# burchim/AVEC

Measured on AMD Instinct MI355X. Metric: AV utterances/sec fwd+bwd (audio T=400, video 100x88x88), higher is better.
Workload: dtype bf16

## Files before the change

avec_amd/csrc/api.hip:

```cpp
#include "common.h"
#include "avec_hip.h"
#include "vec.h"
#include "host_tables.h"
#include <stdarg.h>
#include <stdio.h>

static thread_local char g_err[512] = "";

void avec_set_error(const char* fmt, ...) {
  va_list ap; va_start(ap, fmt); vsnprintf(g_err, sizeof(g_err), fmt, ap); va_end(ap);
}
extern "C" const char* avec_last_error() { return g_err; }

static thread_local char g_kname[128] = "";
void avec_note_kernel(const char* fmt, ...) {
  va_list ap; va_start(ap, fmt); vsnprintf(g_kname, sizeof(g_kname), fmt, ap); va_end(ap);
}
extern "C" const char* avec_last_kernel() { return g_kname; }
extern "C" int avec_version() { return AVEC_ABI_VERSION; }
extern "C" int avec_struct_size(int which) {
  switch (which) {
    case 0: return (int)sizeof(avec_rows_t); case 1: return (int)sizeof(avec_epilogue_t); case 2: return (int)sizeof(avec_attn_t); case 3: return (int)sizeof(avec_tn_item_t);
    case 4: return (int)sizeof(avec_tn_batched_t); case 5: return (int)sizeof(avec_ln_item_t); case 6: return (int)sizeof(avec_fp8_item_t); case 7: return (int)sizeof(avec_wgrad3x3_item_t);
    case 8: return (int)sizeof(avec_ngram_t);
    default: return -1;
  }
}

static WsRegistry g_ws;
static LdsOptin g_lds;

extern "C" int avec_set_reduce_workspace(void* base, long long bytes) {
  int dev = 0; hipError_t e = hipGetDevice(&dev);
  AVEC_CHECK_ARG(e == hipSuccess && dev >= 0 && dev < WsRegistry::MAX_DEV, "set_reduce_workspace: no current device");
  AVEC_CHECK_ARG((base == nullptr && bytes == 0) || (base != nullptr && bytes >= (1 << 16) && ((size_t)base & 255) == 0),
                 "set_reduce_workspace: need a 256-byte aligned buffer of at least 64 KB (or NULL, 0 to unregister)");
  g_ws.set_default(dev, base, (size_t)bytes);
  return 0;
}
extern "C" int avec_set_reduce_workspace_stream(void* base, long long bytes, hipStream_t stream) {
  int dev = 0; hipError_t e = hipGetDevice(&dev);
  AVEC_CHECK_ARG(e == hipSuccess && dev >= 0 && dev < WsRegistry::MAX_DEV && base != nullptr && bytes >= (1 << 16) && ((size_t)base & 255) == 0, "set_reduce_workspace_stream: bad arguments");
  AVEC_CHECK_ARG(g_ws.set_stream(dev, stream, base, (size_t)bytes), "set_reduce_workspace_stream: at most %d stream-bound workspaces", WsRegistry::MAX_STREAMS);
  return 0;
}
ColWs avec_reduce_ws(size_t partial_floats, hipStream_t st) {
  int dev = 0; if (hipGetDevice(&dev) != hipSuccess) return ColWs{nullptr};
  return ColWs{(float*)g_ws.find(dev, st, partial_floats * sizeof(float))};
}

int avec_lds_optin_quiet(const void* kernel, size_t bytes) {
  if (bytes <= LdsOptin::FREE_BYTES) return 0;
  int dev = 0; if (hipGetDevice(&dev) != hipSuccess || dev < 0) return (int)hipErrorNoDevice;
  return g_lds.request(dev, kernel, bytes, [](const void* k, size_t n) {
    const hipError_t e = hipFuncSetAttribute(k, hipFuncAttributeMaxDynamicSharedMemorySize, (int)n);
    if (e != hipSuccess) (void)hipGetLastError();
    return (int)e;
// ... 9 lines not shown
```

avec_amd/lib.py:

```python
import ctypes
import os
import re

_HERE = os.path.dirname(os.path.abspath(__file__))
HEADER = os.path.join(os.path.dirname(_HERE), "include", "avec_hip.h")
LIB_PATH = os.environ.get("AVEC_LIB_PATH") or os.path.join(_HERE, "libavec_hip.so")

F32, BF16 = 0, 1
ROWS_PLAIN, ROWS_CONV_FWD, ROWS_CONV_BWD, ROWS_STEM3D = 0, 1, 2, 3
ACT_NONE, ACT_SWISH, ACT_RELU, ACT_GELU = 0, 1, 2, 3


class Rows(ctypes.Structure):
    _fields_ = [("ld", ctypes.c_longlong), ("rows_out", ctypes.c_int), ("rows_in", ctypes.c_int), ("step", ctypes.c_int),
                ("H", ctypes.c_int), ("W", ctypes.c_int), ("C", ctypes.c_int), ("KH", ctypes.c_int), ("KW", ctypes.c_int),
                ("stride", ctypes.c_int), ("pad", ctypes.c_int), ("OH", ctypes.c_int), ("OW", ctypes.c_int), ("T3", ctypes.c_int)]


class Epilogue(ctypes.Structure):
    _fields_ = [("out", ctypes.c_void_p), ("ldo", ctypes.c_longlong), ("out_f32", ctypes.c_int),
                ("out_pre", ctypes.c_void_p), ("ldpre", ctypes.c_longlong),
                ("bias", ctypes.c_void_p), ("act", ctypes.c_int),
                ("drop_p", ctypes.c_float), ("rng", ctypes.c_void_p), ("rng_stream", ctypes.c_uint),
                ("res", ctypes.c_void_p), ("ldres", ctypes.c_longlong), ("alpha", ctypes.c_float), ("res_act", ctypes.c_int),
# ... 14 lines not shown
                ("de", ctypes.c_void_p), ("ldde", ctypes.c_longlong), ("pbuf", ctypes.c_void_p), ("dsbuf", ctypes.c_void_p), ("ldt", ctypes.c_longlong), ("dsrel", ctypes.c_void_p), ("ldr", ctypes.c_longlong),
                ("B", ctypes.c_int), ("H", ctypes.c_int), ("T", ctypes.c_int), ("d", ctypes.c_int), ("scale", ctypes.c_float), ("Tk", ctypes.c_int)]


class TnItem(ctypes.Structure):
    _fields_ = [("P", ctypes.c_void_p), ("Q", ctypes.c_void_p), ("O", ctypes.c_void_p), ("p_colsum", ctypes.c_void_p),
                ("ldp", ctypes.c_longlong), ("ldq", ctypes.c_longlong), ("ldo", ctypes.c_longlong), ("M", ctypes.c_longlong),
                ("I", ctypes.c_int), ("J", ctypes.c_int), ("q_rows_out", ctypes.c_int), ("q_rows_in", ctypes.c_int), ("q_step", ctypes.c_int),
                ("reserved", ctypes.c_int)]


class TnBatched(ctypes.Structure):
    _fields_ = [("P", ctypes.c_void_p), ("ldp", ctypes.c_longlong), ("Q", ctypes.c_void_p), ("ldq", ctypes.c_longlong),
                ("O", ctypes.c_void_p), ("O_act", ctypes.c_void_p), ("ldo", ctypes.c_longlong),
                ("M", ctypes.c_longlong), ("I", ctypes.c_int), ("J", ctypes.c_int), ("nb_outer", ctypes.c_int), ("nb_inner", ctypes.c_int),
                ("strides6", ctypes.POINTER(ctypes.c_longlong))]


class LnItem(ctypes.Structure):
    _fields_ = [("dy", ctypes.c_void_p), ("x", ctypes.c_void_p), ("mean", ctypes.c_void_p), ("rstd", ctypes.c_void_p), ("dgamma", ctypes.c_void_p),
                ("dbeta", ctypes.c_void_p), ("M", ctypes.c_longlong), ("D", ctypes.c_int), ("dy_f32", ctypes.c_int)]


class Fp8Item(ctypes.Structure):
    _fields_ = [("src", ctypes.c_void_p), ("dst", ctypes.c_void_p), ("n", ctypes.c_longlong), ("slot", ctypes.c_int), ("K", ctypes.c_int), ("Kp", ctypes.c_int),
                ("reserved", ctypes.c_int)]


class WgradItem(ctypes.Structure):
    _fields_ = [("x", ctypes.c_void_p), ("dy", ctypes.c_void_p), ("dw", ctypes.c_void_p), ("images", ctypes.c_longlong), ("C", ctypes.c_int), ("H", ctypes.c_int),
                ("W", ctypes.c_int), ("reserved", ctypes.c_int)]


class NGram(ctypes.Structure):
    _fields_ = [("order", ctypes.c_int), ("V", ctypes.c_int), ("unigram", ctypes.c_void_p), ("ctx_cap", ctypes.c_longlong), ("ctx_key", ctypes.c_void_p),
                ("ctx_bo", ctypes.c_void_p), ("ctx_off", ctypes.c_void_p), ("ctx_cnt", ctypes.c_void_p), ("cont_tok", ctypes.c_void_p), ("cont_lp", ctypes.c_void_p)]


TN_GROUP_MAX, LN_GROUP_MAX, WGRAD_GROUP_MAX = 32, 40, 16
ABI_STRUCTS = (Rows, Epilogue, Attn, TnItem, TnBatched, LnItem, Fp8Item, WgradItem, NGram)


def _ctype(decl):
    decl = decl.strip()
    if "*" in decl or decl.startswith("hipStream_t"):
        return ctypes.c_void_p
    base = re.sub(r"\b[A-Za-z_][A-Za-z_0-9]*$", "", decl).strip() or decl
    base = base.replace("const", "").strip()
    return {"int": ctypes.c_int, "long long": ctypes.c_longlong, "float": ctypes.c_float, "unsigned": ctypes.c_uint,
            "void": None}[base]


def declared_functions(header=HEADER):
    txt = open(header).read()
    txt = re.sub(r"/\*.*?\*/", " ", txt, flags=re.S)
    out = {}
    for m in re.finditer(r"(?:^|\n)\s*(const char\*|long long|int)\s+(avec_[a-z0-9_]+)\s*\(([^;{]*?)\)\s*;", txt):
        ret, name, args = m.group(1), m.group(2), m.group(3)
        args = " ".join(args.split())
        argtypes = [] if args in ("", "void") else [_ctype(a) for a in args.split(",")]
        restype = {"int": ctypes.c_int, "long long": ctypes.c_longlong, "const char*": ctypes.c_char_p}[ret]
        out[name] = (restype, argtypes)
    return out


class _Lib:
    def __init__(self):
        self._dll = None

    def load(self):
        if self._dll is None:
            if not os.path.exists(LIB_PATH):
                raise RuntimeError("libavec_hip.so not found at %s -- build it with `python -m avec_amd.build` "
# ... 32 lines not shown
```

avec_amd/ops.py:

```python
import ctypes
import os

import torch

from . import fp8
from . import runtime as rt
from .lib import (ACT_GELU, ACT_NONE, ACT_RELU, ACT_SWISH, BF16, LN_GROUP_MAX, ROWS_CONV_BWD, ROWS_CONV_FWD, ROWS_PLAIN, ROWS_STEM3D, TN_GROUP_MAX, WGRAD_GROUP_MAX, Attn, Epilogue, LnItem, Rows, TnBatched, TnItem,
                  WgradItem, lib)

_byref = ctypes.byref


class KernelTimer:
    NAMES = {(0, ROWS_CONV_FWD): "gemm_nt<conv_fwd>", (0, ROWS_CONV_BWD): "gemm_nt<conv_bwd_data>", (0, ROWS_STEM3D): "gemm_nt<stem3d>",
             (0, ROWS_PLAIN): "gemm_nt<plain>", (1, ROWS_CONV_FWD): "gemm_tn<conv_wgrad>", (1, ROWS_STEM3D): "gemm_tn<stem3d_wgrad>",
             (1, ROWS_PLAIN): "gemm_tn<plain>", (2, 0): "conv3x3_slab<fwd>", (2, 1): "conv3x3_slab<bwd_data>", (2, 2): "conv3x3_slab<wgrad>"}

    def __init__(self):
        self.enabled = False
        self.records = []

    def reset(self, enabled):
        self.enabled, self.records = enabled, []

    def start(self):
        e = torch.cuda.Event(enable_timing=True)
        e.record()
        return e

    def stop(self, e0, key, flops, abytes=0.0):
        e1 = torch.cuda.Event(enable_timing=True)
        e1.record()
        name = lib.raw("avec_last_kernel")()
        self.records.append((key, flops, e0, e1, name.decode() if name else "", float(abytes)))

    def bracket_overhead_us(self, n=200):
        evs = []
        for _ in range(n):
            a, b = torch.cuda.Event(enable_timing=True), torch.cuda.Event(enable_timing=True)
            a.record(); b.record()
            evs.append((a, b))
# ... 147 lines not shown
    if res is not None:
        ep.res, ep.ldres, ep.res_act, ep.res_cls0 = res.data_ptr(), (N if ldres is None else ldres), int(res_act), int(res_cls0)
        if res_mask is not None:
            ep.res_mask = res_mask.data_ptr()
    ep.alpha = alpha
    if dact_z is not None:
        ep.dact_z, ep.ldz, ep.dact = dact_z.data_ptr(), N, dact
    ep.colsum, ep.stats = _p(colsum), _p(stats)
    if bnb is not None:
        ep.bnb_y, ep.ldby, ep.stats = bnb.y.data_ptr(), N, bnb.stats.data_ptr()
        if bnb.mask_z is not None:
            ep.dact_z, ep.ldz, ep.dact, ep.bnb_mask = bnb.mask_z.data_ptr(), N, 2, 0
        else:
            ep.bnb_ss, ep.bnb_mask = bnb.ss.data_ptr(), 1
    if rows is None:
        rows = rows_plain(K)
    ev = KERNEL_TIMER.start() if KERNEL_TIMER.enabled else None
    lib.gemm_nt(rt.dt() if dtype is None else dtype, A.data_ptr(), _byref(rows), mode, int(a_f32), W.data_ptr(),
                K if ldw is None else ldw, M, N, K, _byref(ep), rt.stream())
    if ev is not None:
        esz = A.element_size()
        KERNEL_TIMER.stop(ev, (0, mode), 2.0 * M * N * K if flops is None else flops,
                          ((M * K + N * K) * esz + M * N * (4 if out_f32 else esz)) if abytes is None else abytes)
    return out


DEFER_WGRAD = os.environ.get("AVEC_DEFER_WGRAD", "1") != "0"
_TN_WHY = False
_TN_FLUSH_AT = TN_GROUP_MAX
_DEFER = {"queues": {}, "task": -1}


class _PendingGrads:
    __slots__ = ("stream", "tn", "ln", "keep", "flops", "cw", "cw_flops", "cw64", "cw64_flops")

    def __init__(self, stream):
        self.stream, self.tn, self.ln, self.keep, self.flops = stream, [], [], [], 0.0
        self.cw, self.cw_flops = [], 0.0
        self.cw64, self.cw64_flops = [], 0.0


def _in_backward():
    return DEFER_WGRAD and torch._C._current_graph_task_id() != -1


def reset_backward_state():
    for q in _DEFER["queues"].values():
        q.tn, q.ln, q.keep, q.flops, q.cw, q.cw_flops, q.cw64, q.cw64_flops = [], [], [], 0.0, [], 0.0, [], 0.0
    _DEFER["task"] = -1
    _PREP_READY["task"], _PREP_READY["m"] = -1, {}
    _LN2_READY["task"], _LN2_READY["m"] = -1, {}
    for ent in _POS_CACHE.values():
        ent[1].de_all, ent[1].remaining = None, ent[1].L


def _pending():
    st = torch.cuda.current_stream()
    q = _DEFER["queues"].get(st.cuda_stream)
    if q is None:
        q = _DEFER["queues"][st.cuda_stream] = _PendingGrads(st)
    task = torch._C._current_graph_task_id()
    if _DEFER["task"] != task:
        if _DEFER["task"] != -1:
            for old in _DEFER["queues"].values():
                old.tn, old.ln, old.keep, old.flops, old.cw, old.cw_flops, old.cw64, old.cw64_flops = [], [], [], 0.0, [], 0.0, [], 0.0
        _DEFER["task"] = task
        torch.autograd.Variable._execution_engine.queue_callback(_flush_at_end)
    return q


def _launch_pending(q, part=None):
    cur = torch.cuda.current_stream()
    if cur.cuda_stream != q.stream.cuda_stream:
        for t in q.keep:
            t.record_stream(cur)
    if q.tn and part in (None, "tn"):
        ev = KERNEL_TIMER.start() if KERNEL_TIMER.enabled else None
        for i in range(0, len(q.tn), TN_GROUP_MAX):
            chunk = q.tn[i:i + TN_GROUP_MAX]
            lib.gemm_tn_grouped(BF16, (TnItem * len(chunk))(*chunk), len(chunk), rt.stream())
        if ev is not None:
            KERNEL_TIMER.stop(ev, (1, ROWS_PLAIN), q.flops, sum(2.0 * it.M * (it.I + it.J) + 4.0 * it.I * it.J for it in q.tn))
        q.tn, q.flops = [], 0.0
    if q.ln and part in (None, "ln"):
        for i in range(0, len(q.ln), LN_GROUP_MAX):
            chunk = q.ln[i:i + LN_GROUP_MAX]
            lib.layernorm_param_grads_grouped(rt.dt(), (LnItem * len(chunk))(*chunk), len(chunk), rt.stream())
        q.ln = []
    if q.cw and part in (None, "cw"):
        ev = KERNEL_TIMER.start() if KERNEL_TIMER.enabled else None
        for i in range(0, len(q.cw), WGRAD_GROUP_MAX):
            chunk = q.cw[i:i + WGRAD_GROUP_MAX]
            lib.wgrad3x3_c128_grouped((WgradItem * len(chunk))(*chunk), len(chunk), rt.stream())
        if ev is not None:
            KERNEL_TIMER.stop(ev, (2, 2), q.cw_flops, sum(2.0 * 2 * it.images * it.H * it.W * it.C + 4.0 * 9 * it.C * it.C for it in q.cw))
        q.cw, q.cw_flops = [], 0.0
    if q.cw64 and part in (None, "cw"):
        ev = KERNEL_TIMER.start() if KERNEL_TIMER.enabled else None
        for i in range(0, len(q.cw64), WGRAD_GROUP_MAX):
            chunk = q.cw64[i:i + WGRAD_GROUP_MAX]
            lib.wgrad3x3_c64_grouped((WgradItem * len(chunk))(*chunk), len(chunk), rt.stream())
        if ev is not None:
            KERNEL_TIMER.stop(ev, (2, 2), q.cw64_flops, sum(2.0 * 2 * it.images * it.H * it.W * it.C + 4.0 * 9 * it.C * it.C for it in q.cw64))
        q.cw64, q.cw64_flops = [], 0.0
    if not q.tn and not q.ln and not q.cw and not q.cw64:
        q.keep = []


def flush_param_grads(all_streams=False):
    if all_streams:
        for q in list(_DEFER["queues"].values()):
            _launch_pending(q)
        return
    q = _DEFER["queues"].get(torch.cuda.current_stream().cuda_stream)
    if q is not None:
        _launch_pending(q)


def _flush_at_end():
    _DEFER["task"] = -1
    flush_param_grads(all_streams=True)


def gemm_tn(P, Q, O, M, I, J, *, ldp=None, q_rows=None, q_mode=ROWS_PLAIN, q_f32=False, ldo=None, dtype=None, p_colsum=None, side=False):
    if q_rows is None:
        q_rows = rows_plain(J)
    if side and q_mode == ROWS_PLAIN and q_f32 and CAST_DEFER and dtype is None and rt.compute_dtype() == "bf16" and _in_backward() and Q.dim() == 2 and Q.dtype == torch.float32:
        Qb = empty((Q.shape[0], J), rt.act_dtype(), Q)
        lib.cast_rows(rt.dt(), Q.data_ptr(), q_rows.ld, Qb.data_ptr(), J, Q.shape[0], J, rt.stream())
        Q, q_f32, q_rows = Qb, False, rows_plain(J, q_rows.rows_out, q_rows.rows_in, q_rows.step)
    if side and q_mode == ROWS_PLAIN and not q_f32 and dtype is None and rt.compute_dtype() == "bf16" and _in_backward():
        it = TnItem()
        it.P, it.Q, it.O, it.p_colsum = P.data_ptr(), Q.data_ptr(), O.data_ptr(), _p(p_colsum)
        it.ldp, it.ldq, it.ldo, it.M, it.I, it.J = (I if ldp is None else ldp), q_rows.ld, (J if ldo is None else ldo), M, I, J
        it.q_rows_out, it.q_rows_in, it.q_step = q_rows.rows_out, q_rows.rows_in, q_rows.step
        if lib.raw("avec_gemm_tn_grouped_ok")(BF16, _byref(it)) and _chunk_readable(P, it.ldp, I, M) and _chunk_readable(Q, it.ldq, J, M):
            q = _pending()
            q.tn.append(it)
# ... 997 lines not shown
        ctx.saved = (grad, M)
        return mean

    @staticmethod
    def backward(ctx, dloss):
        grad, M = ctx.saved
        out = torch.empty_like(grad)
        lib.scale_by_scalar(grad.data_ptr(), dloss.float().contiguous().data_ptr(), 1.0 / M, out.data_ptr(), grad.numel(), rt.stream())
        return out, None, None


def conv2d_fwd(x, weight, N, H, W, Cin, stride, stats=None):
    Cout, KH, KW = weight.shape[0], weight.shape[2], weight.shape[3]
    pad = (KH - 1) // 2
    OH, OW = (H - 1) // stride + 1, (W - 1) // stride + 1
    M = N * OH * OW
    sh = rt.shadow(weight)
    y = empty((M, Cout), rt.act_dtype(), x)
    if _slab_conv(H, W, Cin, Cout, KH, KW, stride):
        ev = KERNEL_TIMER.start() if KERNEL_TIMER.enabled else None
        lib.conv3x3_c64(x.data_ptr(), sh.fwd.data_ptr(), y.data_ptr(), None, _p(stats), N, H, W, 0, rt.stream())
        if ev is not None:
            KERNEL_TIMER.stop(ev, (2, 0), 2.0 * M * Cout * KH * KW * Cin, 2.0 * (N * H * W * Cin + Cout * KH * KW * Cin + M * Cout))
        return y, OH, OW
    gemm_nt(x, sh.fwd, y, M, Cout, KH * KW * Cin, rows=rows_conv(H, W, Cin, KH, KW, stride, pad, OH, OW), mode=ROWS_CONV_FWD, stats=stats,
            abytes=2.0 * (N * H * W * Cin + Cout * KH * KW * Cin + M * Cout))
    return y, OH, OW


SLAB_CONV = True
SLAB_WGRAD128 = True
SHORTCUT_SUBGRID = True
GROUP_WGRAD128 = True


def _slab_conv(H, W, Cin, Cout, KH, KW, stride):
    return SLAB_CONV and rt.act_dtype() == torch.bfloat16 and bool(lib.raw("avec_conv3x3_c64_supported")(H, W, Cin, Cout, KH, KW, stride))


class BnbFuse:
    __slots__ = ("y", "ss", "mask_z", "stats", "done")

    def __init__(self, y, ss, mask_z, C):
        self.y, self.ss, self.mask_z, self.done = y, ss, mask_z, False
        self.stats = rt.zeros_scratch(BNState.NREP * 2 * C, y.device)


BNB_FUSE = False


def conv2d_bwd(dy, x, weight, N, H, W, Cin, stride, OH, OW, need_dx=True, dx_res=None, bnb=None, dx_res_cls0=False, dx_res_mask=None):
    Cout, KH, KW = weight.shape[0], weight.shape[2], weight.shape[3]
    pad = (KH - 1) // 2
    M = N * OH * OW
    sh = rt.shadow(weight)
    if _slab_conv(H, W, Cin, Cout, KH, KW, stride) and H * (W + 1) <= 512:
        if GROUP_WGRAD128 and _in_backward():
            it = WgradItem()
            it.x, it.dy, it.dw, it.images, it.C, it.H, it.W = x.data_ptr(), dy.data_ptr(), grad_of(weight).data_ptr(), N, Cin, H, W
            q = _pending()
            q.cw64.append(it)
            q.keep += [x, dy]
            q.cw64_flops += 2.0 * M * Cout * KH * KW * Cin
        else:
            ev = KERNEL_TIMER.start() if KERNEL_TIMER.enabled else None
            lib.wgrad3x3_c64(x.data_ptr(), dy.data_ptr(), grad_of(weight).data_ptr(), N, H, W, rt.stream())
            if ev is not None:
                KERNEL_TIMER.stop(ev, (2, 2), 2.0 * M * Cout * KH * KW * Cin)
    elif SLAB_CONV and SLAB_WGRAD128 and rt.act_dtype() == torch.bfloat16 and bool(lib.raw("avec_wgrad3x3_c128_supported")(H, W, Cin, Cout, KH, KW, stride)):
        if GROUP_WGRAD128 and _in_backward():
            it = WgradItem()
            it.x, it.dy, it.dw, it.images, it.C, it.H, it.W = x.data_ptr(), dy.data_ptr(), grad_of(weight).data_ptr(), N, Cin, H, W
            q = _pending()
            q.cw.append(it)
            q.keep += [x, dy]
            q.cw_flops += 2.0 * M * Cout * KH * KW * Cin
        else:
            ev = KERNEL_TIMER.start() if KERNEL_TIMER.enabled else None
            lib.wgrad3x3_c128(x.data_ptr(), dy.data_ptr(), grad_of(weight).data_ptr(), N, Cin, H, W, rt.stream())
            if ev is not None:
                KERNEL_TIMER.stop(ev, (2, 2), 2.0 * M * Cout * KH * KW * Cin)
    else:
        gemm_tn(dy, x, grad_of(weight), M, Cout, KH * KW * Cin, q_rows=rows_conv(H, W, Cin, KH, KW, stride, pad, OH, OW), q_mode=ROWS_CONV_FWD, side=True)
    if not need_dx:
        return None
    dx = empty((N * H * W, Cin), rt.act_dtype(), dy)
    if _slab_conv(H, W, Cin, Cout, KH, KW, stride):
        ev = KERNEL_TIMER.start() if KERNEL_TIMER.enabled else None
        if dx_res_mask is not None:
            lib.conv3x3_c64_res_masked(dy.data_ptr(), sh.bwd.data_ptr(), dx.data_ptr(), dx_res.data_ptr(), dx_res_mask.data_ptr(), N, H, W, 1, rt.stream())
        else:
            lib.conv3x3_c64(dy.data_ptr(), sh.bwd.data_ptr(), dx.data_ptr(), _p(dx_res), None, N, H, W, 1, rt.stream())
        if ev is not None:
            KERNEL_TIMER.stop(ev, (2, 1), 2.0 * N * H * W * Cin * KH * KW * Cout, 2.0 * (2 * N * H * W * Cin + Cout * KH * KW * Cin + M * Cout))
        return dx
    fuse = bnb if (bnb is not None and BNB_FUSE and rt.act_dtype() == torch.bfloat16 and Cin % 4 == 0) else None
    gemm_nt(dy, sh.bwd, dx, N * H * W, Cin, KH * KW * Cout, rows=rows_conv(H, W, Cout, KH, KW, stride, pad, OH, OW), mode=ROWS_CONV_BWD,
            res=dx_res, res_act=True, flops=2.0 * N * OH * OW * Cout * KH * KW * Cin, bnb=fuse, res_cls0=dx_res_cls0, res_mask=dx_res_mask,
            abytes=2.0 * (N * H * W * Cin * (2 if dx_res is not None else 1) + Cout * KH * KW * Cin + M * Cout))
    if fuse is not None:
        fuse.done = True
    return dx


RES_MASK = True


def res_mask_ok(H, W, Cin, Cout, stride):
    if rt.act_dtype() != torch.bfloat16 or stride != 1 or Cin != Cout:
        return False
    return _slab_conv(H, W, Cin, Cout, 3, 3, 1) or (Cin >= 128 and Cin % 32 == 0 and W <= 31)


class ResNetBlockFn(torch.autograd.Function):
# ... 467 lines not shown
```

include/avec_hip.h:

```cpp
#ifndef AVEC_HIP_H
#define AVEC_HIP_H
#include <stdint.h>
#ifdef __HIPCC__
#include <hip/hip_runtime.h>
#else
typedef struct ihipStream_t* hipStream_t;
#endif
#ifdef __cplusplus
extern "C" {
#endif

#define AVEC_F32 0
#define AVEC_BF16 1
#define AVEC_ABI_VERSION 4
#define AVEC_STAT_REPLICAS 64

int avec_version(void);
int avec_struct_size(int which);
const char* avec_last_error(void);
const char* avec_last_kernel(void);
int avec_set_reduce_workspace(void* base, long long bytes);
int avec_set_reduce_workspace_stream(void* base, long long bytes, hipStream_t stream);

enum { AVEC_ROWS_PLAIN = 0, AVEC_ROWS_CONV_FWD = 1, AVEC_ROWS_CONV_BWD = 2 };
// ... 166 lines not shown
                        const float* count_ptr, float count, int phase, float* dw, float* dbias, float* dgamma, float* dbeta,
                        int B, int n_mels, int F, int C, hipStream_t stream);
int avec_stem_im2col(int dtype, const float* video, void* A, long long clips, int T, int H, int W, int ldk, hipStream_t stream);
int avec_stem3d_supported(long long clips, int T, int H, int W);
int avec_stem3d_fwd(const float* video, const void* w_shadow, int ldw, const float* bias, void* y, float* stats, long long clips, int T, int H, int W, hipStream_t stream);
int avec_stem3d_wgrad(const float* video, const void* dy, float* dw, long long clips, int T, int H, int W, hipStream_t stream);
int avec_stem3p_supported(long long clips, int T, int H, int W);
int avec_stem3p_fwd(const void* video_bf16, const void* w_shadow, const float* bias, const float* gamma, void* zp, unsigned char* idx, float* stats,
                    long long clips, int T, int H, int W, hipStream_t stream);
int avec_stem3p_reduce(void* dpool, const void* zp, const float* ss, float* dstats, long long frames, int PH, int PW, hipStream_t stream);
int avec_stem3p_wgrad_supported(long long clips, int T, int H, int W);
int avec_stem3p_wgrad(const void* video_bf16, const void* w_shadow, const float* bias, const void* dpool_masked, const unsigned char* idx, const float* ss,
                      const float* gamma, const float* dstats, const float* count_ptr, float count, float* dw, float* dgamma, float* dbeta,
                      long long clips, int T, int H, int W, hipStream_t stream);
int avec_stem3p_dz(const void* video_bf16, const void* w_shadow, const float* bias, const void* dpool_masked, const unsigned char* idx, const float* ss,
                   const float* gamma, const float* dstats, const float* count_ptr, float count, void* dz, float* dgamma, float* dbeta,
                   long long clips, int T, int H, int W, hipStream_t stream);
int avec_stem_pool_fwd(int dtype, const void* y, const float* ss, void* out, unsigned char* idx, void* ymax, long long frames, int H, int W, int C, hipStream_t stream);
int avec_stem_pool_bwd_reduce_pooled(int dtype, const void* dpool, const unsigned char* idx, const void* ymax, const float* ss, float* dstats,
                                     long long frames, int H, int W, int C, hipStream_t stream);
int avec_stem_pool_bwd(int dtype, const void* dpool, const unsigned char* idx, const void* y, const float* ss, const float* gamma, float* dstats,
                       const float* count_ptr, float count, int phase, void* dy, float* dgamma, float* dbeta, long long frames, int H, int W, int C, hipStream_t stream);

int avec_conv3x3_c64_supported(int H, int W, int Cin, int Cout, int KH, int KW, int stride);
int avec_conv3x3_c64(const void* x, const void* w, void* y, const void* res, float* stats, long long images, int H, int W, int flip, hipStream_t stream);
int avec_conv3x3_c64_res_masked(const void* x, const void* w, void* y, const void* res, const unsigned char* res_mask, long long images, int H, int W, int flip, hipStream_t stream);
int avec_wgrad3x3_c64(const void* x, const void* dy, float* dw, long long images, int H, int W, hipStream_t stream);
int avec_wgrad3x3_c128_supported(int H, int W, int Cin, int Cout, int KH, int KW, int stride);
int avec_wgrad3x3_c128(const void* x, const void* dy, float* dw, long long images, int C, int H, int W, hipStream_t stream);
#define AVEC_WGRAD_GROUP_MAX 16
typedef struct { const void* x; const void* dy; float* dw; long long images; int C, H, W, reserved; } avec_wgrad3x3_item_t;
int avec_wgrad3x3_c128_grouped(const avec_wgrad3x3_item_t* items, int n, hipStream_t stream);
int avec_wgrad3x3_c64_grouped(const avec_wgrad3x3_item_t* items, int n, hipStream_t stream);

int avec_video_input(const unsigned char* clips, const long long* clip_off, const int* geom, const int* masks, int max_masks, int channels, const float* lut, float mean, float stdv,
                     int mean_frame, float* out, float* frame_ws, int B, int Tout, int OH, int OW, hipStream_t stream);

long long avec_ctc_workspace_floats(int B, int T, int Lmax);
int avec_ctc_loss(const float* logits, const long long* in_lens, const long long* targets, const long long* tgt_lens, float* nll, float* mean_out,
                  float* grad, float* workspace, int B, int T, int V, int Lmax, int blank, int zero_infinity, hipStream_t stream);
int avec_ctc_loss_multi_fits(int T, int V, int Lmax);
int avec_ctc_loss_multi(int n_heads, const float* const* logits, const long long* const* in_lens, const int* T, float* const* nll, float* const* mean_out, float* const* grad,
                        const long long* targets, const long long* tgt_lens, const float* weights, float* total, int B, int V, int Lmax, int blank, int zero_infinity, hipStream_t stream);
int avec_scale_by_scalar(const float* g, const float* scalar_dev, float mul, float* out, long long n, hipStream_t stream);
int avec_scale_by_scalar_multi(int n_tensors, const float* const* g, float* const* out, const long long* numel, const float* mul, const float* scalar_dev, hipStream_t stream);
int avec_softmax_ce(const float* logits, const long long* targets, long long ignore_index, float* loss, float* mean_out, float* grad, long long M, int V, hipStream_t stream);
int avec_len_affine(const long long* in, long long* out, int n, long long sub, long long div, long long add, hipStream_t stream);
int avec_argmax_rows(const float* x, long long* out, long long M, int V, hipStream_t stream);

typedef struct avec_ngram {
  int order;
  int V;
  const float* unigram;
  long long ctx_cap;
  const unsigned long long* ctx_key;
  const float* ctx_bo;
  const int* ctx_off;
  const int* ctx_cnt;
  const int* cont_tok;
  const float* cont_lp;
} avec_ngram_t;
long long avec_ctc_beam_workspace_bytes(int B, int T, int W);
int avec_ctc_beam_search(const float* logits, const long long* lengths, int B, int T, int V, int W, float inv_tmp, const avec_ngram_t* lm, float alpha, float beta,
                         float oov_logprob, void* workspace, long long workspace_bytes, int* tokens, int* out_len, float* score, float* ctc_logp, hipStream_t stream);
int avec_ngram_rows(const avec_ngram_t* lm, const int* ctx, const int* ctx_len, int n, int max_len, float oov_logprob, float* rows, hipStream_t stream);
long long avec_ctc_align_workspace_bytes(int B, int T, int Lmax);
// ... 26 lines not shown
```

Before: 1869.

## Add grouped MFMA weight-gradient kernel for stride-2 3x3 convolutions

Adds a dedicated bf16 MFMA kernel that computes weight gradients for stride-2 3x3 convs (ResNet downsample layers at 22/11/6 spatial sizes). It loads dy and the four parity-class x windows into double-buffered LDS with global_load_lds, applies boundary masks per tap, and atomically accumulates into fp32 dw. The grads are deferred and batched into a single grouped launch that balances tiles across 256 blocks. This replaces the generic implicit-GEMM TN path for these layers, at the cost of atomics and a narrow supported geometry.

```diff
diff --git a/avec_amd/csrc/api.hip b/avec_amd/csrc/api.hip
--- a/avec_amd/csrc/api.hip
+++ b/avec_amd/csrc/api.hip
@@ -22,7 +22,7 @@
   switch (which) {
     case 0: return (int)sizeof(avec_rows_t); case 1: return (int)sizeof(avec_epilogue_t); case 2: return (int)sizeof(avec_attn_t); case 3: return (int)sizeof(avec_tn_item_t);
     case 4: return (int)sizeof(avec_tn_batched_t); case 5: return (int)sizeof(avec_ln_item_t); case 6: return (int)sizeof(avec_fp8_item_t); case 7: return (int)sizeof(avec_wgrad3x3_item_t);
-    case 8: return (int)sizeof(avec_ngram_t);
+    case 8: return (int)sizeof(avec_ngram_t); case 9: return (int)sizeof(avec_wgrad_s2_item_t);
     default: return -1;
   }
 }
diff --git a/avec_amd/csrc/wgrad_s2.hip b/avec_amd/csrc/wgrad_s2.hip
--- /dev/null
+++ b/avec_amd/csrc/wgrad_s2.hip
@@ -0,0 +1,251 @@
+#include "common.h"
+#include "avec_hip.h"
+#include "wgrad_s2_plan.h"
+
+#include <stdlib.h>
+
+namespace {
+
+typedef __attribute__((ext_vector_type(16))) float ws_f32x16;
+typedef __attribute__((ext_vector_type(8))) __bf16 ws_bf16x8;
+typedef short ws_v4s __attribute__((ext_vector_type(4)));
+typedef __attribute__((address_space(3))) char ws_lds;
+
+constexpr int WS_DYB = WS2_BM * WS2_BCO * 2;
+constexpr int WS_XWB = WS2_WR * WS2_BCI * 2;
+constexpr int WS_TBL = WS_DYB + 4 * WS_XWB;
+constexpr int WS_STAGE = (WS_TBL + 5 * WS2_BM * 2 + 1023) / 1024 * 1024;
+constexpr size_t WS_LDS = 2 * (size_t)WS_STAGE;
+static_assert(WS_LDS <= 160 * 1024, "two stages must fit the LDS");
+constexpr int WS_XI = WS_XWB / 1024, WS_DYI = WS_DYB / 1024;
+constexpr int WS_WAVES = 8, WS_WCO = 4;
+constexpr int WS_NF = WS2_BCO / 32 / WS_WCO;
+static_assert(WS_NF >= 1 && WS2_BCI / 32 * WS_WCO == WS_WAVES, "wave grid");
+
+struct Ws2Item { const char* x; const char* dy; float* dw; Ws2Geom g; int tiles, kinds, nci, L; };
+struct Ws2Group { Ws2Item it[AVEC_WGRAD_GROUP_MAX]; long long cum[AVEC_WGRAD_GROUP_MAX + 1]; int n; };
+
+__device__ __forceinline__ void ws_glds16(unsigned voff, const void* sbase, unsigned lds_dst_uniform) {
+  unsigned keep;
+  asm volatile("s_mov_b32 %0, m0\n\ts_mov_b32 m0, %3\n\ts_nop 0\n\tglobal_load_lds_dwordx4 %1, %2\n\ts_mov_b32 m0, %0" : "=&s"(keep) : "v"(voff), "s"(sbase), "s"(lds_dst_uniform) : "memory");
+}
+__device__ __forceinline__ uint2 ws_tr(const ws_lds* p) {
+  typedef __attribute__((address_space(3))) ws_v4s* lp_t;
+  return __builtin_bit_cast(uint2, __builtin_amdgcn_ds_read_tr16_b64_v4i16((lp_t)p));
+}
+typedef unsigned ws_u32x4 __attribute__((ext_vector_type(4)));
+__device__ __forceinline__ ws_u32x4 ws_ld128(const ws_lds* p) { return *(const __attribute__((address_space(3))) ws_u32x4*)p; }
+struct WsFrag { uint2 lo, hi; };
+__device__ __forceinline__ void ws_and(WsFrag& f, const ws_u32x4& m) { f.lo.x &= m.x; f.lo.y &= m.y; f.hi.x &= m.z; f.hi.y &= m.w; }
+__device__ __forceinline__ ws_f32x16 ws_mma(const WsFrag& a, const WsFrag& b, ws_f32x16 c) {
+  chunk16 fa, fb; fa.w[0] = a.lo.x; fa.w[1] = a.lo.y; fa.w[2] = a.hi.x; fa.w[3] = a.hi.y; fb.w[0] = b.lo.x; fb.w[1] = b.lo.y; fb.w[2] = b.hi.x; fb.w[3] = b.hi.y;
+  return __builtin_amdgcn_mfma_f32_32x32x16_bf16(__builtin_bit_cast(ws_bf16x8, fa), __builtin_bit_cast(ws_bf16x8, fb), c, 0, 0, 0);
+}
+
+struct WsMasks { ws_u32x4 v, t, l, b, r; };
+template <bool ODD>
+__device__ __forceinline__ void ws_load_masks(WsMasks& m, const ws_lds* const tb, const int s) {
+  m.v = ws_ld128(tb + 32 * s); m.t = ws_ld128(tb + 128 + 32 * s); m.l = ws_ld128(tb + 256 + 32 * s);
+  if (ODD) { m.b = ws_ld128(tb + 384 + 32 * s); m.r = ws_ld128(tb + 512 + 32 * s); }
+}
+
+template <bool ODD>
+__device__ __forceinline__ void ws2_run(const char* const xb, const char* const dyb, float* const dw, const Ws2Geom& g, const int nci, ws_lds* const lds, const unsigned lds0,
+                                        const int kind, const int tb, const int te) {
+  const int tid = threadIdx.x, lane = tid & 63, wave = __builtin_amdgcn_readfirstlane(tid >> 6);
+  const int cog = kind / nci, cig = kind - cog * nci, co0 = cog * WS2_BCO, ci0 = cig * WS2_BCI;
+  const int wco = wave % WS_WCO, wci = wave / WS_WCO;
+  const int g4 = lane >> 4, t = lane & 15;
+
+  unsigned aA[WS_NF], aB[9];
+  {
+    const int krow = 8 * (g4 >> 1) + (t >> 2);
+#pragma unroll
+    for (int f = 0; f < WS_NF; ++f) aA[f] = (unsigned)(krow * 256 + (((2 * (WS_NF * wco + f) + (g4 & 1)) ^ (2 * (krow & 3))) << 5) + (t & 3) * 8);
+#pragma unroll
+    for (int tap = 0; tap < 9; ++tap) {
+      const int kh = tap / 3, kw = tap % 3, cls = ((kh + 1) & 1) * 2 + ((kw + 1) & 1);
+      const int row = WS2_HALO + krow - (kh == 0 ? g.OW : 0) - (kw == 0 ? 1 : 0);
+      aB[tap] = (unsigned)(WS_DYB + cls * WS_XWB + row * 128 + (((2 * wci + (g4 & 1)) ^ (2 * ((row >> 1) & 1))) << 5) + (t & 3) * 8);
+    }
+  }
+  const unsigned tblo = (unsigned)(WS_TBL + 16 * (lane >> 5));
+
+  ws_f32x16 acc[WS_NF][9];
+#pragma unroll
+  for (int f = 0; f < WS_NF; ++f)
+#pragma unroll
+    for (int j = 0; j < 9; ++j)
+#pragma unroll
+      for (int r = 0; r < 16; ++r) acc[f][j][r] = 0.f;
+
+  auto issue_stage = [&](const int tile, const int par) {
+    const unsigned m0 = (unsigned)tile * WS2_BM, st = (unsigned)par * WS_STAGE;
+#pragma unroll
+    for (int k = 0; k < WS_DYI / WS_WAVES; ++k) {
+      const int q = wave + WS_WAVES * k, row = 4 * q + (lane >> 4), lu = (lane & 15) ^ (4 * (lane >> 4));
+      unsigned p = m0 + (unsigned)row; p = p < g.P ? p : g.P - 1;
+      ws_glds16((p * (unsigned)g.Cout + (unsigned)(co0 + lu * 8)) * 2u, dyb, lds0 + st + (unsigned)q * 1024u);
+    }
+#pragma unroll
+    for (int k = 0; k < (WS_XI + WS_WAVES - 1) / WS_WAVES; ++k) {
+      const int idx = wave + WS_WAVES * k;
+      if (idx < WS_XI) {
+        int row, lu; ws2_x_slot(idx, lane, row, lu);
+        const unsigned base = ws2_x_base(g, m0, row, lu, ci0);
+#pragma unroll
+        for (int cls = 0; cls < 4; ++cls) ws_glds16(ws2_x_issue(g, base, cls), xb, lds0 + st + (unsigned)(WS_DYB + cls * WS_XWB) + (unsigned)idx * 1024u);
+      }
+    }
+    if (tid < WS2_BM) {
+      const unsigned p = m0 + (unsigned)tid, pc = p < g.P ? p : g.P - 1;
+      const unsigned tt = ws2_div(pc, g.OW), j = pc - tt * (unsigned)g.OW, i = tt - ws2_div(tt, g.OH) * (unsigned)g.OH;
+      typedef __attribute__((address_space(3))) unsigned short lds_u16;
+      lds_u16* const tb_ = (lds_u16*)(lds + st + WS_TBL);
+      tb_[tid] = p < g.P ? 0xffffu : 0u;
+      tb_[WS2_BM + tid] = i > 0 ? 0xffffu : 0u;
+      tb_[2 * WS2_BM + tid] = j > 0 ? 0xffffu : 0u;
+      tb_[3 * WS2_BM + tid] = (int)(2 * i + 1) < g.H ? 0xffffu : 0u;
+      tb_[4 * WS2_BM + tid] = (int)(2 * j + 1) < g.W ? 0xffffu : 0u;
+    }
+  };
+
+  int par = 0;
+  issue_stage(tb, 0);
+  for (int tile = tb; tile < te; ++tile, par ^= 1) {
+    asm volatile("s_waitcnt vmcnt(0) lgkmcnt(0)" ::: "memory");
+    __builtin_amdgcn_s_barrier();
+    asm volatile("" ::: "memory");
+    if (tile + 1 < te) issue_stage(tile + 1, par ^ 1);
+    const ws_lds* const sb = lds + par * WS_STAGE;
+    constexpr int NK = WS2_BM / 16, NSEQ = NK * 9, AHEAD = 3;
+    const ws_lds* const tbl = sb + tblo;
+    WsFrag A[2][WS_NF], B[4]; ws_u32x4 mv[2], mt, ml, mb, mr;
+    auto load_a = [&](const int s) {
+#pragma unroll
+      for (int f = 0; f < WS_NF; ++f) { A[s & 1][f].lo = ws_tr(sb + aA[f] + s * 4096); A[s & 1][f].hi = ws_tr(sb + aA[f] + s * 4096 + 1024); }
+      mv[s & 1] = ws_ld128(tbl + 32 * s);
+    };
+    auto load_b = [&](const int n) { const int s = n / 9, tap = n % 9; B[n & 3].lo = ws_tr(sb + aB[tap] + s * 2048); B[n & 3].hi = ws_tr(sb + aB[tap] + s * 2048 + 512); };
+    load_a(0);
+    mt = ws_ld128(tbl + 128); ml = ws_ld128(tbl + 256);
+#pragma unroll
+    for (int n = 0; n < AHEAD; ++n) load_b(n);
+#pragma unroll
+    for (int n = 0; n < NSEQ; ++n) {
+      const int s = n / 9, tap = n % 9, kh = tap / 3, kw = tap % 3;
+      if (n + AHEAD < NSEQ) load_b(n + AHEAD);
+      if (tap == 4 && s + 1 < NK) load_a(s + 1);
+      if (ODD && tap == 0) { mb = ws_ld128(tbl + 384 + 32 * s); mr = ws_ld128(tbl + 512 + 32 * s); }
+      if (tap == 0) {
+#pragma unroll
+        for (int f = 0; f < WS_NF; ++f) ws_and(A[s & 1][f], mv[s & 1]);
+      }
+      WsFrag& b = B[n & 3];
+      if (kh == 0) ws_and(b, mt);
+      if (kw == 0) ws_and(b, ml);
+      if (ODD && kh == 2) ws_and(b, mb);
+      if (ODD && kw == 2) ws_and(b, mr);
+#pragma unroll
+      for (int f = 0; f < WS_NF; ++f) acc[f][tap] = ws_mma(A[s & 1][f], b, acc[f][tap]);
+      if (tap == 2 && s + 1 < NK) mt = ws_ld128(tbl + 128 + 32 * (s + 1));
+      if (tap == 6 && s + 1 < NK) ml = ws_ld128(tbl + 256 + 32 * (s + 1));
+      __builtin_amdgcn_sched_barrier(0);
+    }
+  }
+#pragma unroll
+  for (int f = 0; f < WS_NF; ++f)
+#pragma unroll
+    for (int j = 0; j < 9; ++j)
+#pragma unroll
+      for (int r = 0; r < 16; ++r) {
+        const int co = co0 + (wco * WS_NF + f) * 32 + (r & 3) + 8 * (r >> 2) + 4 * (lane >> 5), ci = ci0 + wci * 32 + (lane & 31);
+        atomicAdd(dw + ((long long)co * 9 + j) * g.Cin + ci, acc[f][j][r]);
+      }
+  __builtin_amdgcn_s_barrier();
+}
+
+__global__ __launch_bounds__(WS_WAVES * 64) void wgrad3x3_s2_grouped_kernel(Ws2Group grp) {
+  extern __shared__ __attribute__((aligned(16))) char smem[];
+  ws_lds* const lds = (ws_lds*)smem;
+  const unsigned lds0 = (unsigned)(uintptr_t)lds;
+  const long long T = grp.cum[grp.n];
+  const int nb = (int)gridDim.x, per = nb >> 3;
+  const int slot = (nb & 7) ? (int)blockIdx.x : ((int)blockIdx.x & 7) * per + ((int)blockIdx.x >> 3);
+  const long long lo = T * (long long)slot / nb, hi = T * (long long)(slot + 1) / nb;
+  for (int i = 0; i < grp.n; ++i) {
+    const long long c0 = grp.cum[i], c1 = grp.cum[i + 1];
+    if (hi <= c0 || lo >= c1) continue;
+    const Ws2Item& a = grp.it[i];
+    const Ws2Geom g = a.g;
+    const int tiles = a.tiles, kinds = a.kinds, L = a.L, nci = a.nci;
+    int u = (int)((lo > c0 ? lo : c0) - c0); const int u1 = (int)((hi < c1 ? hi : c1) - c0);
+    while (u < u1) {
+      const int r = u / (kinds * L), v = u - r * kinds * L;
+      const int len = tiles - r * L < L ? tiles - r * L : L;
+      const int k = v / len, off = v - k * len;
+      int take = len - off; if (take > u1 - u) take = u1 - u;
+      const int tb = r * L + off;
+      if ((g.H | g.W) & 1) ws2_run<true>(a.x, a.dy, a.dw, g, nci, lds, lds0, k, tb, tb + take);
+      else ws2_run<false>(a.x, a.dy, a.dw, g, nci, lds, lds0, k, tb, tb + take);
+      u += take;
+    }
+  }
+}
+
+bool ws2_geometry(int H, int W) { return (H == 22 && W == 22) || (H == 11 && W == 11) || (H == 6 && W == 6); }
+
+int ws2_geom(const avec_wgrad_s2_item_t& t, Ws2Geom& g) {
+  g.H = t.H; g.W = t.W; g.OH = (t.H + 1) / 2; g.OW = (t.W + 1) / 2; g.Cin = t.Cin; g.Cout = t.Cout;
+  const long long P = t.images * g.OH * g.OW, xbytes = t.images * t.H * t.W * t.Cin * 2;
+  if (t.images <= 0 || P + WS2_WR >= (1ll << 31) || P * t.Cout * 2 >= (1ll << 32) || xbytes + (long long)(t.W + 1) * t.Cin * 2 >= (1ll << 32)) return -1;
+  g.P = (unsigned)P; g.xlast = (unsigned)(xbytes - 16);
+  return 0;
+}
+
+}
+
+extern "C" int avec_wgrad3x3_s2_supported(int H, int W, int Cin, int Cout, int KH, int KW, int stride) {
+  static const bool off = getenv("AVEC_NO_WGRAD_S2") != nullptr;
+  return !off && KH == 3 && KW == 3 && stride == 2 && ws2_geometry(H, W) && Cin >= WS2_BCI && Cin % WS2_BCI == 0 && Cout >= WS2_BCO && Cout % WS2_BCO == 0 && Cin <= 4096 && Cout <= 4096;
+}
+
+extern "C" int avec_wgrad3x3_s2_grouped(const avec_wgrad_s2_item_t* items, int n, hipStream_t st) {
+  AVEC_CHECK_ARG(items && n > 0 && n <= AVEC_WGRAD_GROUP_MAX, "wgrad3x3_s2_grouped: 1..%d items", AVEC_WGRAD_GROUP_MAX);
+  Ws2Group grp; grp.n = n; grp.cum[0] = 0;
+  for (int i = 0; i < n; ++i) {
+    const avec_wgrad_s2_item_t& t = items[i];
+    AVEC_CHECK_ARG(t.x && t.dy && t.dw, "wgrad3x3_s2_grouped: null buffer in item %d", i);
+    AVEC_CHECK_ARG(avec_wgrad3x3_s2_supported(t.H, t.W, t.Cin, t.Cout, 3, 3, 2), "wgrad3x3_s2_grouped: item %d: %d -> %d channels on %dx%d images is not supported", i, t.Cin, t.Cout, t.H, t.W);
+    AVEC_CHECK_ARG((((uintptr_t)t.x | (uintptr_t)t.dy) & 15) == 0 && ((uintptr_t)t.dw & 3) == 0, "wgrad3x3_s2_grouped: item %d: x / dy must be 16-byte aligned", i);
+    Ws2Item& a = grp.it[i]; a.x = (const char*)t.x; a.dy = (const char*)t.dy; a.dw = t.dw;
+    AVEC_CHECK_ARG(ws2_geom(t, a.g) == 0, "wgrad3x3_s2_grouped: item %d too large", i);
+    a.tiles = (int)((a.g.P + WS2_BM - 1) / WS2_BM); a.nci = t.Cin / WS2_BCI; a.kinds = (t.Cout / WS2_BCO) * a.nci;
+    grp.cum[i + 1] = grp.cum[i] + (long long)a.kinds * a.tiles;
+    AVEC_CHECK_ARG(grp.cum[i + 1] < (1ll << 30), "wgrad3x3_s2_grouped: too many tiles");
+  }
+  const long long U = grp.cum[n];
+  const int grid = (int)(U < 256 ? U : 256);
+  const int share = (int)((U + grid - 1) / grid);
+  for (int i = 0; i < n; ++i) grp.it[i].L = share < grp.it[i].tiles ? share : grp.it[i].tiles;
+  if (int r = avec_lds_optin(wgrad3x3_s2_grouped_kernel, WS_LDS)) return r;
+  avec_note_kernel("wgrad3x3_s2_grouped_kernel");
+  hipLaunchKernelGGL(wgrad3x3_s2_grouped_kernel, dim3((unsigned)grid), dim3(WS_WAVES * 64), WS_LDS, st, grp);
+  AVEC_LAUNCH_CHECK();
+  return 0;
+}
+
+extern "C" int avec_wgrad3x3_s2_gather_plan(long long images, int H, int W, int Cin, int Cout, long long tile, int cig, unsigned* out) {
+  AVEC_CHECK_ARG(out && avec_wgrad3x3_s2_supported(H, W, Cin, Cout, 3, 3, 2), "wgrad3x3_s2_gather_plan: unsupported geometry");
+  avec_wgrad_s2_item_t t; t.x = t.dy = nullptr; t.dw = nullptr; t.images = images; t.Cin = Cin; t.Cout = Cout; t.H = H; t.W = W;
+  Ws2Geom g;
+  AVEC_CHECK_ARG(ws2_geom(t, g) == 0, "wgrad3x3_s2_gather_plan: too large");
+  AVEC_CHECK_ARG(tile >= 0 && tile * WS2_BM < (long long)g.P && cig >= 0 && cig < Cin / WS2_BCI, "wgrad3x3_s2_gather_plan: no such tile / chunk");
+  for (int cls = 0; cls < 4; ++cls)
+    for (int idx = 0; idx < WS_XI; ++idx)
+      for (int lane = 0; lane < 64; ++lane) {
+        int row, lu; ws2_x_slot(idx, lane, row, lu);
+        out[(cls * WS2_WR + row) * 8 + (lane & 7)] = ws2_x_issue(g, ws2_x_base(g, (unsigned)(tile * WS2_BM), row, lu, cig * WS2_BCI), cls);
+      }
+  return 0;
+}
diff --git a/avec_amd/csrc/wgrad_s2_plan.h b/avec_amd/csrc/wgrad_s2_plan.h
--- /dev/null
+++ b/avec_amd/csrc/wgrad_s2_plan.h
@@ -0,0 +1,35 @@
+#pragma once
+
+#if defined(__HIPCC__)
+#define WS2_HD __host__ __device__ __forceinline__
+#else
+#define WS2_HD inline
+#endif
+
+constexpr int WS2_BM = 64;
+constexpr int WS2_HALO = 16;
+constexpr int WS2_WR = WS2_BM + WS2_HALO;
+constexpr int WS2_BCO = 128, WS2_BCI = 64;
+
+struct Ws2Geom { int H, W, OH, OW, Cin, Cout; unsigned P, xlast; };
+
+WS2_HD unsigned ws2_div(unsigned p, int d) {
+  switch (d) { case 11: return p / 11u; case 6: return p / 6u; case 3: return p / 3u; default: return p / (unsigned)d; }
+}
+
+WS2_HD unsigned ws2_x_base(const Ws2Geom& g, unsigned m0, int wr, int lu, int ci0) {
+  int pws = (int)m0 + wr - WS2_HALO; pws = pws < 0 ? 0 : pws;
+  const unsigned pw = (unsigned)pws >= g.P ? g.P - 1 : (unsigned)pws;
+  const unsigned t = ws2_div(pw, g.OW), j = pw - t * (unsigned)g.OW, img = ws2_div(t, g.OH), i = t - img * (unsigned)g.OH;
+  return (((img * (unsigned)g.H + 2 * i) * (unsigned)g.W + 2 * j) * (unsigned)g.Cin + (unsigned)(ci0 + lu * 8)) * 2u;
+}
+
+WS2_HD unsigned ws2_x_issue(const Ws2Geom& g, unsigned base, int cls) {
+  const unsigned o = base + (unsigned)(((cls >> 1) * g.W + (cls & 1)) * g.Cin) * 2u;
+  return o < g.xlast ? o : g.xlast;
+}
+
+WS2_HD void ws2_x_slot(int idx, int lane, int& row, int& lu) {
+  row = 8 * idx + (lane >> 3);
+  lu = (lane & 7) ^ (4 * ((row >> 1) & 1));
+}
diff --git a/avec_amd/lib.py b/avec_amd/lib.py
--- a/avec_amd/lib.py
+++ b/avec_amd/lib.py
@@ -70,13 +70,18 @@
                 ("W", ctypes.c_int), ("reserved", ctypes.c_int)]
 
 
+class WgradS2Item(ctypes.Structure):
+    _fields_ = [("x", ctypes.c_void_p), ("dy", ctypes.c_void_p), ("dw", ctypes.c_void_p), ("images", ctypes.c_longlong), ("Cin", ctypes.c_int), ("Cout", ctypes.c_int),
+                ("H", ctypes.c_int), ("W", ctypes.c_int)]
+
+
 class NGram(ctypes.Structure):
     _fields_ = [("order", ctypes.c_int), ("V", ctypes.c_int), ("unigram", ctypes.c_void_p), ("ctx_cap", ctypes.c_longlong), ("ctx_key", ctypes.c_void_p),
                 ("ctx_bo", ctypes.c_void_p), ("ctx_off", ctypes.c_void_p), ("ctx_cnt", ctypes.c_void_p), ("cont_tok", ctypes.c_void_p), ("cont_lp", ctypes.c_void_p)]
 
 
 TN_GROUP_MAX, LN_GROUP_MAX, WGRAD_GROUP_MAX = 32, 40, 16
-ABI_STRUCTS = (Rows, Epilogue, Attn, TnItem, TnBatched, LnItem, Fp8Item, WgradItem, NGram)
+ABI_STRUCTS = (Rows, Epilogue, Attn, TnItem, TnBatched, LnItem, Fp8Item, WgradItem, NGram, WgradS2Item)
 
 
 def _ctype(decl):
diff --git a/avec_amd/ops.py b/avec_amd/ops.py
--- a/avec_amd/ops.py
+++ b/avec_amd/ops.py
@@ -6,7 +6,7 @@
 from . import fp8
 from . import runtime as rt
 from .lib import (ACT_GELU, ACT_NONE, ACT_RELU, ACT_SWISH, BF16, LN_GROUP_MAX, ROWS_CONV_BWD, ROWS_CONV_FWD, ROWS_PLAIN, ROWS_STEM3D, TN_GROUP_MAX, WGRAD_GROUP_MAX, Attn, Epilogue, LnItem, Rows, TnBatched, TnItem,
-                  WgradItem, lib)
+                  WgradItem, WgradS2Item, lib)
 
 _byref = ctypes.byref
 
@@ -220,12 +220,13 @@
 
 
 class _PendingGrads:
-    __slots__ = ("stream", "tn", "ln", "keep", "flops", "cw", "cw_flops", "cw64", "cw64_flops")
+    __slots__ = ("stream", "tn", "ln", "keep", "flops", "cw", "cw_flops", "cw64", "cw64_flops", "cs2", "cs2_flops")
 
     def __init__(self, stream):
         self.stream, self.tn, self.ln, self.keep, self.flops = stream, [], [], [], 0.0
         self.cw, self.cw_flops = [], 0.0
         self.cw64, self.cw64_flops = [], 0.0
+        self.cs2, self.cs2_flops = [], 0.0
 
 
 def _in_backward():
@@ -234,7 +235,7 @@
 
 def reset_backward_state():
     for q in _DEFER["queues"].values():
-        q.tn, q.ln, q.keep, q.flops, q.cw, q.cw_flops, q.cw64, q.cw64_flops = [], [], [], 0.0, [], 0.0, [], 0.0
+        q.tn, q.ln, q.keep, q.flops, q.cw, q.cw_flops, q.cw64, q.cw64_flops, q.cs2, q.cs2_flops = [], [], [], 0.0, [], 0.0, [], 0.0, [], 0.0
     _DEFER["task"] = -1
     _PREP_READY["task"], _PREP_READY["m"] = -1, {}
     _LN2_READY["task"], _LN2_READY["m"] = -1, {}
@@ -251,7 +252,7 @@
     if _DEFER["task"] != task:
         if _DEFER["task"] != -1:
             for old in _DEFER["queues"].values():
-                old.tn, old.ln, old.keep, old.flops, old.cw, old.cw_flops, old.cw64, old.cw64_flops = [], [], [], 0.0, [], 0.0, [], 0.0
+                old.tn, old.ln, old.keep, old.flops, old.cw, old.cw_flops, old.cw64, old.cw64_flops, old.cs2, old.cs2_flops = [], [], [], 0.0, [], 0.0, [], 0.0, [], 0.0
         _DEFER["task"] = task
         torch.autograd.Variable._execution_engine.queue_callback(_flush_at_end)
     return q
@@ -291,7 +292,16 @@
         if ev is not None:
             KERNEL_TIMER.stop(ev, (2, 2), q.cw64_flops, sum(2.0 * 2 * it.images * it.H * it.W * it.C + 4.0 * 9 * it.C * it.C for it in q.cw64))
         q.cw64, q.cw64_flops = [], 0.0
-    if not q.tn and not q.ln and not q.cw and not q.cw64:
+    if q.cs2 and part in (None, "cw"):
+        ev = KERNEL_TIMER.start() if KERNEL_TIMER.enabled else None
+        for i in range(0, len(q.cs2), WGRAD_GROUP_MAX):
+            chunk = q.cs2[i:i + WGRAD_GROUP_MAX]
+            lib.wgrad3x3_s2_grouped((WgradS2Item * len(chunk))(*chunk), len(chunk), rt.stream())
+        if ev is not None:
+            KERNEL_TIMER.stop(ev, (2, 2), q.cs2_flops, sum(2.0 * it.images * (it.H * it.W * it.Cin + ((it.H + 1) // 2) * ((it.W + 1) // 2) * it.Cout) + 4.0 * 9 * it.Cin * it.Cout
+                                                           for it in q.cs2))
+        q.cs2, q.cs2_flops = [], 0.0
+    if not q.tn and not q.ln and not q.cw and not q.cw64 and not q.cs2:
         q.keep = []
 
 
@@ -1355,6 +1365,7 @@
 SLAB_WGRAD128 = True
 SHORTCUT_SUBGRID = True
 GROUP_WGRAD128 = True
+S2_WGRAD = True
 
 
 def _slab_conv(H, W, Cin, Cout, KH, KW, stride):
@@ -1403,6 +1414,14 @@
             lib.wgrad3x3_c128(x.data_ptr(), dy.data_ptr(), grad_of(weight).data_ptr(), N, Cin, H, W, rt.stream())
             if ev is not None:
                 KERNEL_TIMER.stop(ev, (2, 2), 2.0 * M * Cout * KH * KW * Cin)
+    elif (S2_WGRAD and GROUP_WGRAD128 and _in_backward() and rt.act_dtype() == torch.bfloat16 and x.data_ptr() % 16 == 0 and dy.data_ptr() % 16 == 0
+          and bool(lib.raw("avec_wgrad3x3_s2_supported")(H, W, Cin, Cout, KH, KW, stride))):
+        it = WgradS2Item()
+        it.x, it.dy, it.dw, it.images, it.Cin, it.Cout, it.H, it.W = x.data_ptr(), dy.data_ptr(), grad_of(weight).data_ptr(), N, Cin, Cout, H, W
+        q = _pending()
+        q.cs2.append(it)
+        q.keep += [x, dy]
+        q.cs2_flops += 2.0 * M * Cout * KH * KW * Cin
     else:
         gemm_tn(dy, x, grad_of(weight), M, Cout, KH * KW * Cin, q_rows=rows_conv(H, W, Cin, KH, KW, stride, pad, OH, OW), q_mode=ROWS_CONV_FWD, side=True)
     if not need_dx:
diff --git a/include/avec_hip.h b/include/avec_hip.h
--- a/include/avec_hip.h
+++ b/include/avec_hip.h
@@ -222,6 +222,10 @@
 typedef struct { const void* x; const void* dy; float* dw; long long images; int C, H, W, reserved; } avec_wgrad3x3_item_t;
 int avec_wgrad3x3_c128_grouped(const avec_wgrad3x3_item_t* items, int n, hipStream_t stream);
 int avec_wgrad3x3_c64_grouped(const avec_wgrad3x3_item_t* items, int n, hipStream_t stream);
+typedef struct { const void* x; const void* dy; float* dw; long long images; int Cin, Cout, H, W; } avec_wgrad_s2_item_t;
+int avec_wgrad3x3_s2_supported(int H, int W, int Cin, int Cout, int KH, int KW, int stride);
+int avec_wgrad3x3_s2_grouped(const avec_wgrad_s2_item_t* items, int n, hipStream_t stream);
+int avec_wgrad3x3_s2_gather_plan(long long images, int H, int W, int Cin, int Cout, long long tile, int cig, unsigned* out);
 
 int avec_video_input(const unsigned char* clips, const long long* clip_off, const int* geom, const int* masks, int max_masks, int channels, const float* lut, float mean, float stdv,
                      int mean_frame, float* out, float* frame_ws, int B, int Tout, int OH, int OW, hipStream_t stream);
```

Result: no change. 1879 (median of 5 runs) (+0.5%).
